# leggedrobotics/wild_visual_navigation

Measured on AMD Instinct MI355X. Metric: frames/sec (448x448 DINO-ViT-S/8 + seg + MLP train-step), higher is better.
Workload: dtype fp16 + e5m2-MX-correction linears (a w = a_h w_h + 2^-12 (a_h8 w_l8 + a_l8 w_h8); ~16 significand bits per product) + f16 attention products (two-plane q in the first six blocks), fp32 accumulate / residual (<= 1e-3 parity mode)

## Files before the change

### __graft_entry__.py

```python
import os
import sys

ROOT = os.path.dirname(os.path.abspath(__file__))
if ROOT not in sys.path:
    sys.path.insert(0, ROOT)


def build() -> None:
    from wild_visual_navigation_amd.csrc.build import build as build_lib

    path = build_lib(force=False, verbose=True)
    from oracle import build_oracle

    try:
        print("oracle:", build_oracle.build())
    except Exception as e:
        print(f"oracle: C restatement NOT built ({e}); the numpy oracle is used", file=sys.stderr)
    import wild_visual_navigation_amd
    from wild_visual_navigation_amd import _lib

    h = _lib.lib()
    print(f"libwvn_hip version {h.wvn_version()} at {path}; {len(_lib.EXPORTED_SYMBOLS)} entry points bound")


def smoke() -> None:
    import numpy as np
    import torch

    from oracle import interfaces as OI, kmeans_linear as OKL, mlp as OM, segments as OS, vit as OV
    from wild_visual_navigation_amd import ops
    from wild_visual_navigation_amd.backbone import VitBackbone
    from wild_visual_navigation_amd.feature_extractor import FeatureExtractor
    from wild_visual_navigation_amd.model import SimpleMLP
    from wild_visual_navigation_amd.traversability_estimator import MlpTrainer

    assert torch.cuda.is_available(), "smoke() needs a GPU"
    dev = torch.device("cuda:0")
    S, P, heads = 64, 8, 6
    G = S // P
    sd = OV.make_vit_state_dict("vit_small", P, pretrain_grid=4, seed=0, depth=2)
    img = torch.rand(2, 3, S, S, generator=torch.Generator().manual_seed(0))
    ref_tok = OV.vit_tokens(sd, OI.normalize(img), P, heads)[:, 1:]
    frame = torch.randint(0, 256, (1, 3, 90, 120), generator=torch.Generator().manual_seed(4), dtype=torch.uint8)
    ref_frame = OV.vit_tokens(sd, OI.dino_transform(frame.float() / 255, S), P, heads)[:, 1:]
    for prec, tol in (("exact", 1e-3), ("mixed", 1e-3), ("fp32", 1e-3), ("fp16", 8e-3), ("bf16", 6e-2)):
        bb = VitBackbone(sd, S, P, heads, device=dev, precision=prec)
        tok = bb.forward_tokens(img.to(dev)).cpu()
        err = (tok - ref_tok).abs().max().item()
        print(f"smoke: ViT tokens [{prec}] max|err| = {err:.3e} (tol {tol})")
        assert err < tol, f"backbone parity failed in {prec}: {err}"
        err = (bb.forward_tokens(frame.to(dev)).cpu() - ref_frame).abs().max().item()
        assert err < tol, f"fused ingest failed in {prec}: {err}"
    seg = OS.segment_grid(S, S, 16)[0, 0]
    dense = OI.upsample_bilinear_ac(ref_tok.reshape(2, G, G, -1).permute(0, 3, 1, 2), S)
    want = torch.stack([OS.sparsify_features(dense[b:b + 1], seg) for b in range(2)])
    got = ops.segpool_bilinear_mean(seg[None].expand(2, S, S).to(dev), ref_tok.to(dev), G, int(seg.max()) + 1).cpu()
    err = (got - want).abs().max().item()
    print(f"smoke: fused segment pooling max|err| = {err:.3e}")
    assert err < 1e-4
    code = torch.randn(1, G * G, 90, generator=torch.Generator().manual_seed(3))
    lab, _ = ops.kmeans_cosine(code.to(dev), K=5, iters=10, relabel=False)
    want_lab = OI.kmeans_cosine_labels(code[0].numpy(), 5)
    assert np.array_equal(lab[0].cpu().numpy(), want_lab), "k-means labels differ from the oracle"
    labp, _ = ops.kmeans_cosine_pixels(code.to(dev), G, 40, K=5, iters=10, relabel=False, form="direct")
    assert np.array_equal(labp[0].cpu().numpy(), OI.kmeans_cosine_labels_pixels(code[0].numpy(), G, 40, 5)), "pixel k-means labels differ"
    labl, _ = ops.kmeans_cosine_pixels(code.to(dev), G, 40, K=5, iters=10, relabel=False)
    assert np.array_equal(labl[0].cpu().numpy(), OKL.kmeans_cosine_labels_pixels_linear(code[0].numpy(), G, 40, 5)), "linear-form pixel k-means labels differ"
    print("smoke: k-means labels bit-exact (patch and pixel resolution)")
    D = 90
    g = torch.Generator().manual_seed(1)
    x = torch.randn(64, D, generator=g)
    yv = torch.rand(64, generator=g) < 0.3
    y = yv.float() * (0.5 + 0.5 * torch.rand(64, generator=g))
    model = SimpleMLP(D, [256, 32, 1], True)
    sd0 = {k: v.detach().clone() for k, v in model.state_dict().items()}
    model.to(dev)
    tr = MlpTrainer(model)
    st = OM.TrainState(sd0)
    for _ in range(3):
        got_l = tr.train_step(x.to(dev), y.to(dev), yv.to(dev)).cpu()
        want_l = OM.train_step(st, x, y, yv)
    assert abs(got_l[0].item() - want_l["loss_total"]) < 1e-5, (got_l, want_l)
    werr = max((model.state_dict()[k].cpu() - st.sd[k]).abs().max().item() for k in st.sd)
    print(f"smoke: MLP 3 Adam steps loss {got_l[0].item():.6f} (oracle {want_l['loss_total']:.6f}), max|dW| = {werr:.2e}")
    assert werr < 1e-5
    fe = FeatureExtractor(dev, segmentation_type="grid", feature_type="dino", input_size=S, backbone_type="vit_small",
                          patch_size=P, pretrained_weights=sd, precision="bf16")
    edges, feat, segm, center, _ = fe.extract(img[:1].to(dev), cell_size=16)
    assert feat.shape == (16, 384) and segm.shape == (S, S) and edges.shape[0] == 2
    print("smoke: ok")


if __name__ == "__main__":
    build()
    if len(sys.argv) > 1 and sys.argv[1] == "smoke":
        smoke()
```

### wild_visual_navigation_amd/csrc/gemm_n384_x3.hip

```cpp
#include <type_traits>

#include "common.h"
#include "wvn_internal.h"

namespace {

constexpr int NN = 384;
constexpr int NTILE = NN / 32;
constexpr int BKS = 16;
constexpr int BM = 128;
constexpr int NS = 4;
constexpr int W_PLANE = NN * BKS * 2;
constexpr int A_PLANE = BM * BKS * 2;
constexpr int A_OFF = 2 * W_PLANE;
constexpr int STAGE_BYTES = 2 * W_PLANE + 2 * A_PLANE;
constexpr int RING_BYTES = NS * STAGE_BYTES;
constexpr int STG_PITCH = 132;
constexpr int STG_BYTES = 32 * STG_PITCH * 4;
constexpr int BIAS_OFF = RING_BYTES;
constexpr int LS_OFF = BIAS_OFF + NN * 4;
constexpr int LDS_BYTES = LS_OFF + NN * 4;
constexpr int WP = 6, AP = 2;

struct N384X3Params {
// ... 259 lines not shown
    };
    __syncthreads();
#pragma unroll
    for (int j = 0; j < PD; ++j) load_a(j, j);
#pragma unroll
    for (int i0 = 0; i0 < FNS - 1; ++i0)
      if (i0 < nk) {
#pragma unroll
        for (int u = 0; u < FW; ++u) piece_w(i0, u);
      }

    f32x16_t acc[NTILE];
#pragma unroll
    for (int t = 0; t < NTILE; ++t)
#pragma unroll
      for (int r = 0; r < 16; ++r) acc[t][r] = 0.f;

    for (int ib = 0; ib < nk; ib += PD) {
#pragma unroll
      for (int jj = 0; jj < PD; ++jj) {
        const int i = ib + jj;
        long long c0 = 0, c1 = 0;
        if constexpr (TIMING) c0 = (long long)__builtin_amdgcn_s_memtime();
        asm volatile("s_waitcnt vmcnt(%0)" ::"n"((FNS - 2) * FW) : "memory");
        __builtin_amdgcn_s_barrier();
        if constexpr (TIMING) c1 = (long long)__builtin_amdgcn_s_memtime();
        __builtin_amdgcn_sched_barrier(0);
        const unsigned char* st = smem + (i % FNS) * FSTAGE;
        const bf16x8_t ah = __builtin_bit_cast(bf16x8_t, afh[jj]), al = __builtin_bit_cast(bf16x8_t, afl[jj]);
        bf16x8_t wh[2][2], wl[2][2];
#pragma unroll
        for (int t = 0; t < 2; ++t) {
          wh[0][t] = *(const bf16x8_t*)(st + rdw + t * 1024);
          wl[0][t] = *(const bf16x8_t*)(st + rdw + W_PLANE + t * 1024);
        }
#pragma unroll
        for (int pr = 0; pr < NTILE / 2; ++pr) {
          const int cur = pr & 1, nx = cur ^ 1;
          piece_w(i + FNS - 1, pr);
          if (pr + 1 < NTILE / 2) {
#pragma unroll
            for (int t = 0; t < 2; ++t) {
              wh[nx][t] = *(const bf16x8_t*)(st + rdw + (2 * pr + 2 + t) * 1024);
              wl[nx][t] = *(const bf16x8_t*)(st + rdw + W_PLANE + (2 * pr + 2 + t) * 1024);
            }
          }
#pragma unroll
          for (int term = 0; term < 3; ++term)
#pragma unroll
            for (int t = 0; t < 2; ++t) {
              const bf16x8_t w = term == 1 ? wl[cur][t] : wh[cur][t];
              const bf16x8_t a = term == 0 ? al : ah;
              acc[2 * pr + t] = __builtin_amdgcn_mfma_f32_32x32x16_bf16(w, a, acc[2 * pr + t], 0, 0, 0);
            }
#pragma unroll
          for (int n = 0; n < 6; ++n) {
            __builtin_amdgcn_sched_group_barrier(0x008, 1, 0);
            __builtin_amdgcn_sched_group_barrier(0x100, 1, 0);
            __builtin_amdgcn_sched_group_barrier(0x010, 1, 0);
            __builtin_amdgcn_sched_group_barrier(0x002, 2, 0);
          }
          __builtin_amdgcn_sched_barrier(0);
        }
        if (i + PD < nk) load_a(i + PD, jj);
        __builtin_amdgcn_sched_barrier(0);
        if constexpr (TIMING) { t_wait += c1 - c0; t_steps += (long long)__builtin_amdgcn_s_memtime() - c1; }
      }
    }
    long long e0 = 0;
    if constexpr (TIMING) e0 = (long long)__builtin_amdgcn_s_memtime();
    asm volatile("s_waitcnt vmcnt(0)" ::: "memory");
    n384_epilogue(acc, smem, wave, lane, m0w, rs_c, p.ldc, bias_l, ls_l, p.stats, p.eps, p.M, p.pos, p.npatch, p.ntok_s);
    if constexpr (TIMING) t_epi += (long long)__builtin_amdgcn_s_memtime() - e0;
  }
  if constexpr (TIMING) {
    if (lane == 0 && p.dbg) {
      long long* d = p.dbg + ((size_t)blockIdx.x * 4 + wave) * 4;
      d[0] = t_wait; d[1] = t_steps; d[2] = t_epi; d[3] = (long long)__builtin_amdgcn_s_memtime() - t_start;
    }
  }
}

constexpr int PFW = 3;
constexpr int PNS = 6;
constexpr int PRING_BYTES = PNS * FSTAGE;
constexpr int PSTG_PITCH = 68;
constexpr int PSTG_BYTES = 32 * PSTG_PITCH * 4;
constexpr int PBIAS_OFF = PRING_BYTES;
constexpr int PLS_OFF = PBIAS_OFF + NN * 4;
constexpr int PSTAT_OFF = PLS_OFF + NN * 4;
constexpr int PAIR_LDS_BYTES = PSTAT_OFF + 2 * BM * 8;
static_assert(8 * PSTG_BYTES <= PRING_BYTES && PAIR_LDS_BYTES <= 160 * 1024, "staging images must fit in the ring, the whole in the LDS");

__device__ inline void n384_pair_epilogue(const f32x16_t (&acc)[NTILE / 2], unsigned char* smem, int wave, int lane, int rg, int ch, int m0w,
                                          __amdgpu_buffer_rsrc_t rs_c, int ldc, const float* bias_l, const float* ls_l, float* stats, float eps, int M) {
  const int l31 = lane & 31, hi = lane >> 5, l15 = lane & 15, rq = lane >> 4;
  __syncthreads();
  float* stg = (float*)(smem + wave * PSTG_BYTES);
  const unsigned cvoff = (unsigned)((rq * ldc + l15 * 4) * 4);
  const int col0 = 192 * ch;
  float s1[8], s2[8];
#pragma unroll
  for (int it = 0; it < 8; ++it) { s1[it] = 0.f; s2[it] = 0.f; }
#pragma unroll
  for (int c = 0; c < 3; ++c) {
#pragma unroll
    for (int tt = 0; tt < 2; ++tt)
#pragma unroll
      for (int g = 0; g < 4; ++g) {
        const f32x16_t& a = acc[2 * c + tt];
        const f32x4_t o = {a[4 * g], a[4 * g + 1], a[4 * g + 2], a[4 * g + 3]};
        *(f32x4_t*)(stg + l31 * PSTG_PITCH + 32 * tt + 8 * g + 4 * hi) = o;
      }
    const f32x4_t b4 = *(const f32x4_t*)(bias_l + col0 + 64 * c + l15 * 4);
    const f32x4_t l4 = *(const f32x4_t*)(ls_l + col0 + 64 * c + l15 * 4);
    u32x4_t r[8];
    unsigned so_dst[8];
#pragma unroll
    for (int it = 0; it < 8; ++it) {
      so_dst[it] = __builtin_amdgcn_readfirstlane(((m0w + 4 * it) * ldc + col0 + 64 * c) * 4);
      r[it] = __builtin_amdgcn_raw_buffer_load_b128(rs_c, cvoff, so_dst[it], 0);
    }
#pragma unroll
    for (int it = 0; it < 8; ++it) {
      const f32x4_t v = *(const f32x4_t*)(stg + (4 * it + rq) * PSTG_PITCH + l15 * 4);
      u32x4_t o;
#pragma unroll
      for (int e = 0; e < 4; ++e) {
        const float y = (v[e] + b4[e]) * l4[e] + __uint_as_float(r[it][e]);
        o[e] = __float_as_uint(y);
        s1[it] += y;
        s2[it] = fmaf(y, y, s2[it]);
      }
      wvn_store_b128_guarded(o, rs_c, cvoff, so_dst[it]);
    }
  }
  if (stats) {
    float* sx = (float*)(smem + PSTAT_OFF);
    auto dpp_add = [](float v, auto ctrl) {
      constexpr int C = decltype(ctrl)::value;
      return v + __builtin_bit_cast(float, __builtin_amdgcn_update_dpp(0, __builtin_bit_cast(int, v), C, 0xf, 0xf, false));
    };
#pragma unroll
    for (int it = 0; it < 8; ++it) {
      float a = s1[it], b = s2[it];
      a = dpp_add(a, std::integral_constant<int, 0xB1>{}); b = dpp_add(b, std::integral_constant<int, 0xB1>{});
      a = dpp_add(a, std::integral_constant<int, 0x4E>{}); b = dpp_add(b, std::integral_constant<int, 0x4E>{});
      a = dpp_add(a, std::integral_constant<int, 0x141>{}); b = dpp_add(b, std::integral_constant<int, 0x141>{});
      a = dpp_add(a, std::integral_constant<int, 0x140>{}); b = dpp_add(b, std::integral_constant<int, 0x140>{});
      if (l15 == 0) *(wvn_f32x2_t*)(sx + ((size_t)ch * BM + rg * 32 + 4 * it + rq) * 2) = wvn_f32x2_t{a, b};
    }
    __syncthreads();
    if (ch == 0 && lane < 32) {
      const int m = m0w + lane;
      if (m < M) {
        const wvn_f32x2_t p0 = *(const wvn_f32x2_t*)(sx + ((size_t)rg * 32 + lane) * 2), p1 = *(const wvn_f32x2_t*)(sx + ((size_t)BM + rg * 32 + lane) * 2);
        const float a = p0[0] + p1[0], b = p0[1] + p1[1];
        const float mean = a * (1.0f / NN);
        const float var = fmaxf(b * (1.0f / NN) - mean * mean, 0.f);
        *(wvn_f32x2_t*)(stats + 2 * (size_t)m) = wvn_f32x2_t{mean, 1.0f / sqrtf(var + eps)};
      }
    }
  }
}

template <bool TIMING>
__global__ __launch_bounds__(512, 1) void gemm_n384_x3_frag_pair_kernel(N384X3Params p) {
  wvn_fp16_saturate();
  extern __shared__ __attribute__((aligned(16))) unsigned char smem[];
  const int tid = threadIdx.x, lane = tid & 63;
  const int wave = __builtin_amdgcn_readfirstlane(tid >> 6);
  const int rg = wave & 3, ch = wave >> 2;
  const int l31 = lane & 31, hi = lane >> 5;
  const int nk = p.K / BKS;
  const float* bias_l = (const float*)(smem + PBIAS_OFF);
  const float* ls_l = (const float*)(smem + PLS_OFF);
  for (int i = tid; i < NN; i += 512) {
    ((float*)(smem + PBIAS_OFF))[i] = p.bias ? p.bias[i] : 0.f;
    ((float*)(smem + PLS_OFF))[i] = p.ls ? p.ls[i] : 1.f;
  }
  const __amdgpu_buffer_rsrc_t rs_w = __builtin_amdgcn_make_buffer_rsrc((void*)p.W, 0, (unsigned)((size_t)2 * NN * p.K * 2), 0x00020000);
  const size_t mpad = (size_t)(p.M + 31) / 32 * 32;
  const __amdgpu_buffer_rsrc_t rs_a = __builtin_amdgcn_make_buffer_rsrc((void*)p.A, 0, (unsigned)((p.a_plane + mpad * p.K) * 2), 0x00020000);
  const __amdgpu_buffer_rsrc_t rs_c = __builtin_amdgcn_make_buffer_rsrc((void*)p.C, 0, (unsigned)((size_t)p.M * p.ldc * 4), 0x00020000);
  const unsigned wv0 = (unsigned)(wave * PFW * 1024 + lane * 16);
  const unsigned rdw = l31 * 32 + ((hi ^ ((l31 >> 3) & 1)) << 4) + ch * 6 * 1024;
  const unsigned a_lo_off = (unsigned)(p.a_plane * 2);

  long long t_wait = 0, t_steps = 0, t_epi = 0;
  const long long t_start = TIMING ? (long long)__builtin_amdgcn_s_memtime() : 0;
  const int nrb = (p.M + BM - 1) / BM;
  for (int rb = blockIdx.x; rb < nrb; rb += gridDim.x) {
    const int m0w = rb * BM + rg * 32;
    const unsigned a_base = __builtin_amdgcn_readfirstlane((unsigned)((size_t)(m0w >> 5) * nk * 1024));
    auto piece_w = [&](int i, int u) {
      unsigned char* st = smem + (i % PNS) * FSTAGE;
      __builtin_amdgcn_raw_ptr_buffer_load_lds(rs_w, (__attribute__((address_space(3))) void*)(st + (wave * PFW + u) * 1024), 16, wv0 + u * 1024,
                                               __builtin_amdgcn_readfirstlane((unsigned)i * FSTAGE), 0, 0);
    };
    u32x4_t afh[PD], afl[PD];
    auto load_a = [&](int i, int slot) {
      const unsigned so = __builtin_amdgcn_readfirstlane(a_base + (unsigned)i * 1024);
      afh[slot] = __builtin_amdgcn_raw_buffer_load_b128(rs_a, lane * 16, so, 0);
      afl[slot] = __builtin_amdgcn_raw_buffer_load_b128(rs_a, lane * 16, so + a_lo_off, 0);
    };
    __syncthreads();
#pragma unroll
    for (int j = 0; j < PD; ++j) load_a(j, j);
#pragma unroll
    for (int i0 = 0; i0 < PNS - 1; ++i0)
      if (i0 < nk) {
#pragma unroll
        for (int u = 0; u < PFW; ++u) piece_w(i0, u);
      }

    f32x16_t acc[NTILE / 2];
#pragma unroll
    for (int t = 0; t < NTILE / 2; ++t)
#pragma unroll
      for (int r = 0; r < 16; ++r) acc[t][r] = 0.f;

    bf16x8_t wh[2][2], wl[2][2];
    asm volatile("s_waitcnt vmcnt(%0)" ::"n"((PNS - 2) * PFW) : "memory");
    __builtin_amdgcn_s_barrier();
#pragma unroll
    for (int t = 0; t < 2; ++t) {
      wh[0][t] = *(const bf16x8_t*)(smem + rdw + t * 1024);
      wl[0][t] = *(const bf16x8_t*)(smem + rdw + W_PLANE + t * 1024);
    }
    for (int ib = 0; ib < nk; ib += PD) {
#pragma unroll
      for (int jj = 0; jj < PD; ++jj) {
        const int i = ib + jj;
        long long c0 = 0, c1 = 0;
        if constexpr (TIMING) c0 = (long long)__builtin_amdgcn_s_memtime();
        asm volatile("s_waitcnt vmcnt(%0)" ::"n"((PNS - 3) * PFW) : "memory");
        __builtin_amdgcn_s_barrier();
        if constexpr (TIMING) c1 = (long long)__builtin_amdgcn_s_memtime();
        __builtin_amdgcn_sched_barrier(0);
        const unsigned char* st = smem + (i % PNS) * FSTAGE;
        const unsigned char* st1 = smem + ((i + 1) % PNS) * FSTAGE;
        const bf16x8_t ah = __builtin_bit_cast(bf16x8_t, afh[jj]), al = __builtin_bit_cast(bf16x8_t, afl[jj]);
        const int s0 = jj & 1;
#pragma unroll
        for (int pr = 0; pr < NTILE / 4; ++pr) {
          const int cur = (s0 + pr) & 1, nx = cur ^ 1;
          piece_w(i + PNS - 1, pr);
          if (pr + 1 < NTILE / 4) {
#pragma unroll
            for (int t = 0; t < 2; ++t) {
              wh[nx][t] = *(const bf16x8_t*)(st + rdw + (2 * pr + 2 + t) * 1024);
              wl[nx][t] = *(const bf16x8_t*)(st + rdw + W_PLANE + (2 * pr + 2 + t) * 1024);
            }
          } else {
#pragma unroll
            for (int t = 0; t < 2; ++t) {
              wh[nx][t] = *(const bf16x8_t*)(st1 + rdw + t * 1024);
              wl[nx][t] = *(const bf16x8_t*)(st1 + rdw + W_PLANE + t * 1024);
            }
          }
#pragma unroll
          for (int term = 0; term < 3; ++term)
#pragma unroll
            for (int t = 0; t < 2; ++t) {
              const bf16x8_t w = term == 1 ? wl[cur][t] : wh[cur][t];
              const bf16x8_t a = term == 0 ? al : ah;
              acc[2 * pr + t] = __builtin_amdgcn_mfma_f32_32x32x16_bf16(w, a, acc[2 * pr + t], 0, 0, 0);
            }
#pragma unroll
          for (int n = 0; n < 6; ++n) {
            __builtin_amdgcn_sched_group_barrier(0x008, 1, 0);
            __builtin_amdgcn_sched_group_barrier(0x100, 1, 0);
            __builtin_amdgcn_sched_group_barrier(0x010, 1, 0);
            __builtin_amdgcn_sched_group_barrier(0x002, 2, 0);
          }
          __builtin_amdgcn_sched_barrier(0);
        }
        if (i + PD < nk) load_a(i + PD, jj);
        __builtin_amdgcn_sched_barrier(0);
        if constexpr (TIMING) { t_wait += c1 - c0; t_steps += (long long)__builtin_amdgcn_s_memtime() - c1; }
      }
    }
    long long e0 = 0;
    if constexpr (TIMING) e0 = (long long)__builtin_amdgcn_s_memtime();
    asm volatile("s_waitcnt vmcnt(0)" ::: "memory");
    n384_pair_epilogue(acc, smem, wave, lane, rg, ch, m0w, rs_c, p.ldc, bias_l, ls_l, p.stats, p.eps, p.M);
    if constexpr (TIMING) t_epi += (long long)__builtin_amdgcn_s_memtime() - e0;
  }
  if constexpr (TIMING) {
    if (lane == 0 && p.dbg && ch == 0) {
      long long* d = p.dbg + ((size_t)blockIdx.x * 4 + rg) * 4;
      d[0] = t_wait; d[1] = t_steps; d[2] = t_epi; d[3] = (long long)__builtin_amdgcn_s_memtime() - t_start;
    }
  }
}

typedef __attribute__((ext_vector_type(8))) int i32x8_t;
typedef __attribute__((ext_vector_type(8))) _Float16 f16x8_t;
constexpr int MXD = 2;
constexpr int MX_SC_ONE = 0x7f7f7f7f, MX_SC_RES = 0x73737373;

struct N384MXExtra { unsigned a_l8_off; };

template <bool TIMING, int VAR = 0>
__global__ __launch_bounds__(512, 1) void gemm_n384_mx_pair_kernel(N384X3Params p, N384MXExtra ex) {
  wvn_fp16_saturate();
  extern __shared__ __attribute__((aligned(16))) unsigned char smem[];
  const int tid = threadIdx.x, lane = tid & 63;
  const int wave = __builtin_amdgcn_readfirstlane(tid >> 6);
  const int rg = wave & 3, ch = wave >> 2;
  const int l31 = lane & 31, hi = lane >> 5;
  const int nk = p.K / BKS;
  const int nmac = p.K / 64;
  const float* bias_l = (const float*)(smem + PBIAS_OFF);
  const float* ls_l = (const float*)(smem + PLS_OFF);
  for (int i = tid; i < NN; i += 512) {
    ((float*)(smem + PBIAS_OFF))[i] = p.bias ? p.bias[i] : 0.f;
    ((float*)(smem + PLS_OFF))[i] = p.ls ? p.ls[i] : 1.f;
  }
  const __amdgpu_buffer_rsrc_t rs_w = __builtin_amdgcn_make_buffer_rsrc((void*)p.W, 0, (unsigned)((size_t)4 * NN * p.K), 0x00020000);
  const size_t mpad = (size_t)(p.M + 31) / 32 * 32;
  const __amdgpu_buffer_rsrc_t rs_a = __builtin_amdgcn_make_buffer_rsrc((void*)p.A, 0, (unsigned)(ex.a_l8_off + mpad * p.K), 0x00020000);
  const __amdgpu_buffer_rsrc_t rs_c = __builtin_amdgcn_make_buffer_rsrc((void*)p.C, 0, (unsigned)((size_t)p.M * p.ldc * 4), 0x00020000);
  const unsigned wv0 = (unsigned)(wave * PFW * 1024 + lane * 16);
  const unsigned rdw = l31 * 32 + ((hi ^ ((l31 >> 3) & 1)) << 4) + ch * 6 * 1024;

  long long t_wait = 0, t_steps = 0, t_epi = 0;
  const long long t_start = TIMING ? (long long)__builtin_amdgcn_s_memtime() : 0;
  const int nrb = (p.M + BM - 1) / BM;
  for (int rb = blockIdx.x; rb < nrb; rb += gridDim.x) {
    const int m0w = rb * BM + rg * 32;
    const unsigned a_base = __builtin_amdgcn_readfirstlane((unsigned)((size_t)(m0w >> 5) * p.K * 64));
    const unsigned a8_base = __builtin_amdgcn_readfirstlane((unsigned)((size_t)(m0w >> 5) * p.K * 32));
    auto piece_w = [&](int i, int u) {
      unsigned char* st = smem + (i % PNS) * FSTAGE;
      __builtin_amdgcn_raw_ptr_buffer_load_lds(rs_w, (__attribute__((address_space(3))) void*)(st + (wave * PFW + u) * 1024), 16, wv0 + u * 1024,
                                               __builtin_amdgcn_readfirstlane((unsigned)i * FSTAGE), 0, 0);
    };
    u32x4_t ah[MXD][4], a8[MXD][2][2];
    auto load_ah = [&](int c, int slot) {
#pragma unroll
      for (int s = 0; s < 4; ++s)
        ah[slot][s] = __builtin_amdgcn_raw_buffer_load_b128(rs_a, lane * 16, __builtin_amdgcn_readfirstlane(a_base + (unsigned)(c * 4 + s) * 1024), 0);
    };
    auto load_a8 = [&](int c, int slot) {
#pragma unroll
      for (int x = 0; x < 2; ++x)
        a8[slot][1][x] = __builtin_amdgcn_raw_buffer_load_b128(rs_a, lane * 16, __builtin_amdgcn_readfirstlane(a8_base + ex.a_l8_off + (unsigned)(c * 2 + x) * 1024), 0);
    };
    auto derive_h8 = [&](int slot) {
      typedef __attribute__((ext_vector_type(2))) short s16x2_t;
      typedef __attribute__((ext_vector_type(2))) _Float16 h2_t;
#pragma unroll
      for (int sfr = 0; sfr < 4; ++sfr) {
        uint32_t d[2] = {0, 0};
#pragma unroll
        for (int e = 0; e < 4; ++e) {
          const uint32_t pr = ah[slot][sfr][e];
          const s16x2_t o = __builtin_bit_cast(s16x2_t, d[e >> 1]);
          d[e >> 1] = __builtin_bit_cast(uint32_t, (e & 1) ? __builtin_amdgcn_cvt_scalef32_pk_bf8_f16(o, __builtin_bit_cast(h2_t, pr), 1.0f, true)
                                                           : __builtin_amdgcn_cvt_scalef32_pk_bf8_f16(o, __builtin_bit_cast(h2_t, pr), 1.0f, false));
        }
        a8[slot][0][sfr >> 1][2 * (sfr & 1)] = d[0];
        a8[slot][0][sfr >> 1][2 * (sfr & 1) + 1] = d[1];
      }
    };
    __syncthreads();
#pragma unroll
    for (int c = 0; c < MXD; ++c) {
      load_ah(c, c);
      __builtin_amdgcn_sched_barrier(0);
      load_a8(c, c);
      __builtin_amdgcn_sched_barrier(0);
    }
#pragma unroll
    for (int i0 = 0; i0 < PNS - 1; ++i0)
      if (i0 < nk) {
#pragma unroll
        for (int u = 0; u < PFW; ++u) piece_w(i0, u);
      }

    f32x16_t acc[NTILE / 2];
#pragma unroll
    for (int t = 0; t < NTILE / 2; ++t)
#pragma unroll
      for (int r = 0; r < 16; ++r) acc[t][r] = 0.f;

    u32x4_t wq[2][2][2];
    asm volatile("s_waitcnt vmcnt(%0)" ::"n"((PNS - 2) * PFW) : "memory");
    __builtin_amdgcn_s_barrier();
#pragma unroll
    for (int x = 0; x < 2; ++x)
#pragma unroll
      for (int t = 0; t < 2; ++t) wq[0][x][t] = *(const u32x4_t*)(smem + rdw + x * W_PLANE + t * 1024);
    for (int ib = 0; ib < nk; ib += 4 * MXD) {
#pragma unroll
      for (int jj = 0; jj < 4 * MXD; ++jj) {
        const int i = ib + jj;
        const int kind = jj & 3, slot = jj >> 2;
        long long c0 = 0, c1 = 0;
        if constexpr (TIMING) c0 = (long long)__builtin_amdgcn_s_memtime();
        if constexpr (VAR != 4) {
          constexpr int W3 = (PNS - 3) * PFW;
          if (jj == 0) { if (i == 0) asm volatile("s_waitcnt vmcnt(%0)" ::"n"(W3) : "memory"); else asm volatile("s_waitcnt vmcnt(%0)" ::"n"(W3 + 6) : "memory"); }
          else if (jj == 1) { if (i == 1) asm volatile("s_waitcnt vmcnt(%0)" ::"n"(W3) : "memory"); else asm volatile("s_waitcnt vmcnt(%0)" ::"n"(W3 + 2) : "memory"); }
          else if (jj == 2) { if (i == 2) asm volatile("s_waitcnt vmcnt(%0)" ::"n"(W3 + 4) : "memory"); else asm volatile("s_waitcnt vmcnt(%0)" ::"n"(W3 + 6) : "memory"); }
          else if ((jj & 3) == 0) asm volatile("s_waitcnt vmcnt(%0)" ::"n"(W3 + 6) : "memory");
          else if ((jj & 3) == 1) asm volatile("s_waitcnt vmcnt(%0)" ::"n"(W3 + 2) : "memory");
          else if ((jj & 3) == 2) asm volatile("s_waitcnt vmcnt(%0)" ::"n"(W3 + 6) : "memory");
          else asm volatile("s_waitcnt vmcnt(%0)" ::"n"(W3 + 4) : "memory");
          __builtin_amdgcn_s_barrier();
        }
        if constexpr (TIMING) c1 = (long long)__builtin_amdgcn_s_memtime();
        __builtin_amdgcn_sched_barrier(0);
        const unsigned char* st = smem + (i % PNS) * FSTAGE;
        const unsigned char* st1 = smem + ((i + 1) % PNS) * FSTAGE;
        const int s0 = jj & 1;
#pragma unroll
        for (int pr = 0; pr < NTILE / 4; ++pr) {
          const int cur = (s0 + pr) & 1, nx = cur ^ 1;
          if constexpr (!(VAR & 1) || VAR == 4) piece_w(i + PNS - 1, pr);
          const unsigned char* src = pr + 1 < NTILE / 4 ? st + (2 * pr + 2) * 1024 : st1;
#pragma unroll
          for (int x = 0; x < 2; ++x)
#pragma unroll
            for (int t = 0; t < 2; ++t) wq[nx][x][t] = *(const u32x4_t*)(src + rdw + x * W_PLANE + t * 1024);
          if (kind == 1 && pr == 0) derive_h8(slot);
          if (kind < 2) {
#pragma unroll
            for (int x = 0; x < 2; ++x)
#pragma unroll
              for (int t = 0; t < 2; ++t)
                acc[2 * pr + t] = __builtin_amdgcn_mfma_f32_32x32x16_f16(__builtin_bit_cast(f16x8_t, wq[cur][x][t]), __builtin_bit_cast(f16x8_t, ah[slot][2 * kind + x]),
                                                                         acc[2 * pr + t], 0, 0, 0);
#pragma unroll
            for (int n = 0; n < 4; ++n) {
              __builtin_amdgcn_sched_group_barrier(0x008, 1, 0);
              __builtin_amdgcn_sched_group_barrier(0x100, 1, 0);
              __builtin_amdgcn_sched_group_barrier(0x010, 1, 0);
              __builtin_amdgcn_sched_group_barrier(0x002, 2, 0);
            }
          } else {
            const u32x4_t a0 = a8[slot][kind - 2][0], a1 = a8[slot][kind - 2][1];
            const i32x8_t av = {(int)a0[0], (int)a0[1], (int)a0[2], (int)a0[3], (int)a1[0], (int)a1[1], (int)a1[2], (int)a1[3]};
#pragma unroll
            for (int t = 0; t < 2; ++t) {
              const u32x4_t w0 = wq[cur][0][t], w1 = wq[cur][1][t];
              const i32x8_t wv = {(int)w0[0], (int)w0[1], (int)w0[2], (int)w0[3], (int)w1[0], (int)w1[1], (int)w1[2], (int)w1[3]};
              acc[2 * pr + t] = __builtin_amdgcn_mfma_scale_f32_32x32x64_f8f6f4(wv, av, acc[2 * pr + t], 1, 1, 0, kind == 2 ? MX_SC_RES : MX_SC_ONE, 0,
                                                                                kind == 2 ? MX_SC_ONE : MX_SC_RES);
            }
#pragma unroll
            for (int n = 0; n < 2; ++n) {
              __builtin_amdgcn_sched_group_barrier(0x008, 1, 0);
              __builtin_amdgcn_sched_group_barrier(0x100, 2, 0);
              __builtin_amdgcn_sched_group_barrier(0x010, 1, 0);
              __builtin_amdgcn_sched_group_barrier(0x002, 4, 0);
            }
          }
          __builtin_amdgcn_sched_barrier(0);
        }
        const int c2 = (i >> 2) + MXD;
        if constexpr (!(VAR & 2) || VAR == 4) {
          if (kind == 1) load_ah(c2, slot);
          if (kind == 3) load_a8(c2, slot);
        }
        __builtin_amdgcn_sched_barrier(0);
        if constexpr (TIMING) { t_wait += c1 - c0; t_steps += (long long)__builtin_amdgcn_s_memtime() - c1; }
      }
    }
    long long e0 = 0;
    if constexpr (TIMING) e0 = (long long)__builtin_amdgcn_s_memtime();
    asm volatile("s_waitcnt vmcnt(0)" ::: "memory");
    n384_pair_epilogue(acc, smem, wave, lane, rg, ch, m0w, rs_c, p.ldc, bias_l, ls_l, p.stats, p.eps, p.M);
    if constexpr (TIMING) t_epi += (long long)__builtin_amdgcn_s_memtime() - e0;
  }
  if constexpr (TIMING) {
    if (lane == 0 && p.dbg && ch == 0) {
      long long* d = p.dbg + ((size_t)blockIdx.x * 4 + rg) * 4;
      d[0] = t_wait; d[1] = t_steps; d[2] = t_epi; d[3] = (long long)__builtin_amdgcn_s_memtime() - t_start;
    }
  }
}

int g_n384_mx_var = 0;
int g_n384_pair = 1;

int n384x3_num_cus() {
  static int n = 0;
  if (n == 0) {
    int dev = 0;
    hipDeviceProp_t prop;
    if (hipGetDevice(&dev) == hipSuccess && hipGetDeviceProperties(&prop, dev) == hipSuccess) n = prop.multiProcessorCount;
    if (n <= 0) n = 256;
  }
  return n;
}

}

int wvn_gemm_n384_x3_launch(const GemmBf16Params& g, int epi, hipStream_t st) {
  const bool patch = epi == EPI_PATCH;
  if (epi != EPI_RESID_F32 && epi != EPI_ACCUM_F32 && !patch) return WVN_ERR_ARG;
  if (patch && (!g.pos || g.npatch <= 0 || (g.npatch & 1) || g.ntok_s < g.npatch + 1 || g.ldc != NN || g.ls || (g.M % g.npatch) != 0)) return WVN_ERR_ARG;
  if (g.N != NN || g.K <= 0 || (g.K % BKS) != 0 || g.M <= 0 || !g.A || !g.A_lo || !g.W || !g.W_lo || !g.C) return WVN_ERR_ARG;
  if ((g.lda % 8) || (g.ldw % 8) || (g.ldc % 4) || g.ldw != g.K) return WVN_ERR_ARG;
  if (((uintptr_t)g.A | (uintptr_t)g.A_lo | (uintptr_t)g.W | (uintptr_t)g.W_lo | (uintptr_t)g.C) & 15) return WVN_ERR_ARG;
  if (g.A_lo <= g.A || g.W_lo <= g.W) return WVN_ERR_ARG;
  const size_t a_plane = (size_t)(g.A_lo - g.A), w_plane = (size_t)(g.W_lo - g.W);
  const size_t c_rows = patch ? (size_t)(g.M / g.npatch) * g.ntok_s : (size_t)g.M;
  if ((a_plane + (size_t)g.M * g.lda) * 2 >= (1ull << 32) || c_rows * g.ldc * 4 >= (1ull << 32) || (w_plane + (size_t)NN * g.ldw) * 2 >= (1ull << 32))
    return WVN_ERR_ARG;
  N384X3Params p{};
  p.A = g.A; p.a_plane = a_plane; p.lda = g.lda; p.W = g.W; p.w_plane = w_plane; p.ldw = g.ldw; p.bias = g.bias; p.ls = g.ls;
  p.C = (float*)g.C; p.ldc = g.ldc; p.M = g.M; p.K = g.K; p.dbg = g.dbg; p.stats = g.ln_stats_out; p.eps = g.ln_eps;
  if (patch) { p.pos = g.pos; p.npatch = g.npatch; p.ntok_s = g.ntok_s; p.c_rows = (int)c_rows; p.stats = nullptr; }
  static LdsOptIn lds_opt_in;
  if (const int rc = lds_opt_in(LDS_BYTES, (const void*)gemm_n384_x3_kernel<false>, (const void*)gemm_n384_x3_kernel<true>)) return rc;
  const int ncu = n384x3_num_cus(), nrb = ceil_div(g.M, BM);
  const int grid = nrb < ncu ? nrb : ncu;
  if (p.dbg) hipLaunchKernelGGL(gemm_n384_x3_kernel<true>, dim3(grid), dim3(256), LDS_BYTES, st, p);
  else hipLaunchKernelGGL(gemm_n384_x3_kernel<false>, dim3(grid), dim3(256), LDS_BYTES, st, p);
  WVN_LAUNCH_CHECK();
  return WVN_OK;
}

int wvn_gemm_n384_x3_frag_launch(const GemmBf16Params& g, int epi, hipStream_t st) {
  if (epi != EPI_RESID_F32 && epi != EPI_ACCUM_F32) return WVN_ERR_ARG;
  if (g.N != NN || g.K <= 0 || (g.K % (BKS * PD)) != 0 || g.M <= 0 || !g.A || !g.A_lo || !g.W || !g.C || (g.ldc % 4)) return WVN_ERR_ARG;
  if (((uintptr_t)g.A | (uintptr_t)g.A_lo | (uintptr_t)g.W | (uintptr_t)g.C) & 15) return WVN_ERR_ARG;
  if (g.A_lo <= g.A) return WVN_ERR_ARG;
  const size_t a_plane = (size_t)(g.A_lo - g.A), mpad = (size_t)(g.M + 31) / 32 * 32;
  if ((a_plane + mpad * g.K) * 2 >= (1ull << 32) || (size_t)g.M * g.ldc * 4 >= (1ull << 32) || (size_t)2 * NN * g.K * 2 >= (1ull << 31)) return WVN_ERR_ARG;
  N384X3Params p{};
  p.A = g.A; p.a_plane = a_plane; p.lda = g.K; p.W = g.W; p.w_plane = 0; p.ldw = g.K; p.bias = g.bias; p.ls = g.ls;
  p.C = (float*)g.C; p.ldc = g.ldc; p.M = g.M; p.K = g.K; p.dbg = g.dbg; p.stats = g.ln_stats_out; p.eps = g.ln_eps;
  static LdsOptIn lds_opt_in;
  if (const int rc = lds_opt_in(PAIR_LDS_BYTES, (const void*)gemm_n384_x3_frag_kernel<false>, (const void*)gemm_n384_x3_frag_kernel<true>,
                                (const void*)gemm_n384_x3_frag_pair_kernel<false>, (const void*)gemm_n384_x3_frag_pair_kernel<true>)) return rc;
  const int ncu = n384x3_num_cus(), nrb = ceil_div(g.M, BM);
  const int grid = nrb < ncu ? nrb : ncu;
  if (g_n384_pair) {
    if (p.dbg) hipLaunchKernelGGL(gemm_n384_x3_frag_pair_kernel<true>, dim3(grid), dim3(512), PAIR_LDS_BYTES, st, p);
    else hipLaunchKernelGGL(gemm_n384_x3_frag_pair_kernel<false>, dim3(grid), dim3(512), PAIR_LDS_BYTES, st, p);
  } else if (p.dbg) hipLaunchKernelGGL(gemm_n384_x3_frag_kernel<true>, dim3(grid), dim3(256), LDS_BYTES, st, p);
  else hipLaunchKernelGGL(gemm_n384_x3_frag_kernel<false>, dim3(grid), dim3(256), LDS_BYTES, st, p);
  WVN_LAUNCH_CHECK();
  return WVN_OK;
}
int wvn_gemm_n384_mx_launch(const GemmBf16Params& g, int epi, hipStream_t st) {
  if (epi != EPI_RESID_F32 && epi != EPI_ACCUM_F32) return WVN_ERR_ARG;
  if (g.N != NN || g.K <= 0 || (g.K % 128) != 0 || g.M <= 0 || !g.A || !g.A_lo || !g.W || !g.C || (g.ldc % 4)) return WVN_ERR_ARG;
  if (((uintptr_t)g.A | (uintptr_t)g.A_lo | (uintptr_t)g.W | (uintptr_t)g.C) & 15) return WVN_ERR_ARG;
  const size_t mpad = (size_t)(g.M + 31) / 32 * 32;
  const uintptr_t a0 = (uintptr_t)g.A, al = (uintptr_t)g.A_lo;
  if (al < a0 + mpad * g.K * 2) return WVN_ERR_ARG;
  const uintptr_t top = al + mpad * g.K;
  if (top - a0 >= (1ull << 32) || (size_t)g.M * g.ldc * 4 >= (1ull << 32) || (size_t)4 * NN * g.K >= (1ull << 31)) return WVN_ERR_ARG;
  N384X3Params p{};
  p.A = g.A; p.a_plane = 0; p.lda = g.K; p.W = g.W; p.w_plane = 0; p.ldw = g.K; p.bias = g.bias; p.ls = g.ls;
  p.C = (float*)g.C; p.ldc = g.ldc; p.M = g.M; p.K = g.K; p.dbg = g.dbg; p.stats = g.ln_stats_out; p.eps = g.ln_eps;
  N384MXExtra ex{(unsigned)(al - a0)};
  static LdsOptIn lds_opt_in;
  if (const int rc = lds_opt_in(PAIR_LDS_BYTES, (const void*)gemm_n384_mx_pair_kernel<false>, (const void*)gemm_n384_mx_pair_kernel<true>,
                                (const void*)gemm_n384_mx_pair_kernel<true, 1>, (const void*)gemm_n384_mx_pair_kernel<true, 2>,
                                (const void*)gemm_n384_mx_pair_kernel<true, 3>, (const void*)gemm_n384_mx_pair_kernel<true, 4>)) return rc;
  const int ncu = n384x3_num_cus(), nrb = ceil_div(g.M, BM);
  const int grid = nrb < ncu ? nrb : ncu;
  if (p.dbg && g_n384_mx_var == 1) hipLaunchKernelGGL((gemm_n384_mx_pair_kernel<true, 1>), dim3(grid), dim3(512), PAIR_LDS_BYTES, st, p, ex);
  else if (p.dbg && g_n384_mx_var == 2) hipLaunchKernelGGL((gemm_n384_mx_pair_kernel<true, 2>), dim3(grid), dim3(512), PAIR_LDS_BYTES, st, p, ex);
  else if (p.dbg && g_n384_mx_var == 3) hipLaunchKernelGGL((gemm_n384_mx_pair_kernel<true, 3>), dim3(grid), dim3(512), PAIR_LDS_BYTES, st, p, ex);
  else if (p.dbg && g_n384_mx_var == 4) hipLaunchKernelGGL((gemm_n384_mx_pair_kernel<true, 4>), dim3(grid), dim3(512), PAIR_LDS_BYTES, st, p, ex);
  else if (p.dbg) hipLaunchKernelGGL(gemm_n384_mx_pair_kernel<true>, dim3(grid), dim3(512), PAIR_LDS_BYTES, st, p, ex);
  else hipLaunchKernelGGL(gemm_n384_mx_pair_kernel<false>, dim3(grid), dim3(512), PAIR_LDS_BYTES, st, p, ex);
  WVN_LAUNCH_CHECK();
  return WVN_OK;
}
void wvn_gemm_n384_x3_set_pair(int on) {
  if (on >= 16) { g_n384_mx_var = on - 16; return; }
  g_n384_pair = on ? 1 : 0;
}
```

Before: 882.5.

## Overlap next row-block A/W prefetch and residual loads with MX pair GEMM epilogue

Restructures the MX pair GEMM's persistent row-block loop so the last k-trip is peeled. That trip prefetches the residual tile into registers, preloads the first W stages for the next row block into ring slots, and issues the next block's A loads from inside a new custom epilogue after each column group. The epilogue stages through unused ring slots, adds bias/layer-scale/residual and computes LayerNorm stats. This is meant to hide the epilogue's global residual reads and the next tile's pipeline fill latency. It adds many registers and complex vmcnt accounting, and only fully applies when nk is a multiple of the stage count.

```diff
diff --git a/__graft_entry__.py b/__graft_entry__.py
--- a/__graft_entry__.py
+++ b/__graft_entry__.py
@@ -72,6 +72,7 @@
     x = torch.randn(64, D, generator=g)
     yv = torch.rand(64, generator=g) < 0.3
     y = yv.float() * (0.5 + 0.5 * torch.rand(64, generator=g))
+    torch.manual_seed(0)
     model = SimpleMLP(D, [256, 32, 1], True)
     sd0 = {k: v.detach().clone() for k, v in model.state_dict().items()}
     model.to(dev)
diff --git a/wild_visual_navigation_amd/csrc/gemm_n384_x3.hip b/wild_visual_navigation_amd/csrc/gemm_n384_x3.hip
--- a/wild_visual_navigation_amd/csrc/gemm_n384_x3.hip
+++ b/wild_visual_navigation_amd/csrc/gemm_n384_x3.hip
@@ -585,6 +585,78 @@
 
 struct N384MXExtra { unsigned a_l8_off; };
 
+constexpr int MX_STG_OFF = 3 * FSTAGE;
+static_assert(MX_STG_OFF + 8 * PSTG_BYTES <= PRING_BYTES, "the MX staging images must fit in ring slots 3 - 5");
+template <class AfterGroup>
+__device__ inline void n384_mx_pair_epilogue(const f32x16_t (&acc)[NTILE / 2], const u32x4_t (&res)[24], unsigned char* smem, int wave, int lane, int rg, int ch,
+                                             int m0w, __amdgpu_buffer_rsrc_t rs_c, int ldc, const float* bias_l, const float* ls_l, float* stats, float eps, int M,
+                                             AfterGroup&& after_group) {
+  const int l31 = lane & 31, hi = lane >> 5, l15 = lane & 15, rq = lane >> 4;
+  float* stg = (float*)(smem + MX_STG_OFF + wave * PSTG_BYTES);
+  const unsigned cvoff = (unsigned)((rq * ldc + l15 * 4) * 4);
+  const int col0 = 192 * ch;
+  float s1[8], s2[8];
+#pragma unroll
+  for (int it = 0; it < 8; ++it) { s1[it] = 0.f; s2[it] = 0.f; }
+#pragma unroll
+  for (int c = 0; c < 3; ++c) {
+#pragma unroll
+    for (int tt = 0; tt < 2; ++tt)
+#pragma unroll
+      for (int g = 0; g < 4; ++g) {
+        const f32x16_t& a = acc[2 * c + tt];
+        const f32x4_t o = {a[4 * g], a[4 * g + 1], a[4 * g + 2], a[4 * g + 3]};
+        *(f32x4_t*)(stg + l31 * PSTG_PITCH + 32 * tt + 8 * g + 4 * hi) = o;
+      }
+    const f32x4_t b4 = *(const f32x4_t*)(bias_l + col0 + 64 * c + l15 * 4);
+    const f32x4_t l4 = *(const f32x4_t*)(ls_l + col0 + 64 * c + l15 * 4);
+#pragma unroll
+    for (int it = 0; it < 8; ++it) {
+      const unsigned so = __builtin_amdgcn_readfirstlane(((m0w + 4 * it) * ldc + col0 + 64 * c) * 4);
+      const f32x4_t v = *(const f32x4_t*)(stg + (4 * it + rq) * PSTG_PITCH + l15 * 4);
+      u32x4_t o;
+#pragma unroll
+      for (int e = 0; e < 4; ++e) {
+        const float y = (v[e] + b4[e]) * l4[e] + __uint_as_float(res[8 * c + it][e]);
+        o[e] = __float_as_uint(y);
+        s1[it] += y;
+        s2[it] = fmaf(y, y, s2[it]);
+      }
+      wvn_store_b128_guarded(o, rs_c, cvoff, so);
+    }
+    if (c == 0) after_group(std::integral_constant<int, 0>{});
+    if (c == 1) after_group(std::integral_constant<int, 1>{});
+  }
+  if (stats) {
+    float* sx = (float*)(smem + PSTAT_OFF);
+    auto dpp_add = [](float v, auto ctrl) {
+      constexpr int C = decltype(ctrl)::value;
+      return v + __builtin_bit_cast(float, __builtin_amdgcn_update_dpp(0, __builtin_bit_cast(int, v), C, 0xf, 0xf, false));
+    };
+#pragma unroll
+    for (int it = 0; it < 8; ++it) {
+      float a = s1[it], b = s2[it];
+      a = dpp_add(a, std::integral_constant<int, 0xB1>{}); b = dpp_add(b, std::integral_constant<int, 0xB1>{});
+      a = dpp_add(a, std::integral_constant<int, 0x4E>{}); b = dpp_add(b, std::integral_constant<int, 0x4E>{});
+      a = dpp_add(a, std::integral_constant<int, 0x141>{}); b = dpp_add(b, std::integral_constant<int, 0x141>{});
+      a = dpp_add(a, std::integral_constant<int, 0x140>{}); b = dpp_add(b, std::integral_constant<int, 0x140>{});
+      if (l15 == 0) *(wvn_f32x2_t*)(sx + ((size_t)ch * BM + rg * 32 + 4 * it + rq) * 2) = wvn_f32x2_t{a, b};
+    }
+    __syncthreads();
+    if (ch == 0 && lane < 32) {
+      const int m = m0w + lane;
+      if (m < M) {
+        const wvn_f32x2_t p0 = *(const wvn_f32x2_t*)(sx + ((size_t)rg * 32 + lane) * 2), p1 = *(const wvn_f32x2_t*)(sx + ((size_t)BM + rg * 32 + lane) * 2);
+        const float a = p0[0] + p1[0], b = p0[1] + p1[1];
+        const float mean = a * (1.0f / NN);
+        const float var = fmaxf(b * (1.0f / NN) - mean * mean, 0.f);
+        *(wvn_f32x2_t*)(stats + 2 * (size_t)m) = wvn_f32x2_t{mean, 1.0f / sqrtf(var + eps)};
+      }
+    }
+  }
+}
+
+
 template <bool TIMING, int VAR = 0>
 __global__ __launch_bounds__(512, 1) void gemm_n384_mx_pair_kernel(N384X3Params p, N384MXExtra ex) {
   wvn_fp16_saturate();
@@ -607,29 +679,51 @@
   const __amdgpu_buffer_rsrc_t rs_c = __builtin_amdgcn_make_buffer_rsrc((void*)p.C, 0, (unsigned)((size_t)p.M * p.ldc * 4), 0x00020000);
   const unsigned wv0 = (unsigned)(wave * PFW * 1024 + lane * 16);
   const unsigned rdw = l31 * 32 + ((hi ^ ((l31 >> 3) & 1)) << 4) + ch * 6 * 1024;
+  const unsigned cvoff = (unsigned)(((lane >> 4) * p.ldc + (lane & 15) * 4) * 4);
+  const bool pre = (nk % PNS) == 0;
 
   long long t_wait = 0, t_steps = 0, t_epi = 0;
   const long long t_start = TIMING ? (long long)__builtin_amdgcn_s_memtime() : 0;
   const int nrb = (p.M + BM - 1) / BM;
+  unsigned a_base = 0, a8_base = 0;
+  auto set_a_base = [&](int rb_) {
+    const size_t R = (size_t)(rb_ * (BM / 32) + rg);
+    a_base = __builtin_amdgcn_readfirstlane((unsigned)(R * p.K * 64));
+    a8_base = __builtin_amdgcn_readfirstlane((unsigned)(R * p.K * 32));
+  };
+  u32x4_t ah[MXD][4], a8[MXD][2][2];
+  auto load_ah = [&](int c, int slot) {
+#pragma unroll
+    for (int s = 0; s < 4; ++s)
+      ah[slot][s] = __builtin_amdgcn_raw_buffer_load_b128(rs_a, lane * 16, __builtin_amdgcn_readfirstlane(a_base + (unsigned)(c * 4 + s) * 1024), 0);
+  };
+  auto load_a8 = [&](int c, int slot) {
+#pragma unroll
+    for (int x = 0; x < 2; ++x)
+      a8[slot][1][x] = __builtin_amdgcn_raw_buffer_load_b128(rs_a, lane * 16, __builtin_amdgcn_readfirstlane(a8_base + ex.a_l8_off + (unsigned)(c * 2 + x) * 1024), 0);
+  };
+  auto load_a_head = [&](int rb_, int c) {
+    set_a_base(rb_);
+    __builtin_amdgcn_sched_barrier(0);
+    load_ah(c, c);
+    __builtin_amdgcn_sched_barrier(0);
+    load_a8(c, c);
+    __builtin_amdgcn_sched_barrier(0);
+  };
+  static_assert(MXD == 2, "one 64-k step of A behind each of the epilogue's first two column groups");
+  load_a_head(blockIdx.x, 0);
+  load_a_head(blockIdx.x, 1);
   for (int rb = blockIdx.x; rb < nrb; rb += gridDim.x) {
     const int m0w = rb * BM + rg * 32;
-    const unsigned a_base = __builtin_amdgcn_readfirstlane((unsigned)((size_t)(m0w >> 5) * p.K * 64));
-    const unsigned a8_base = __builtin_amdgcn_readfirstlane((unsigned)((size_t)(m0w >> 5) * p.K * 32));
-    auto piece_w = [&](int i, int u) {
+    auto piece_w = [&](int i, int u, int src) {
       unsigned char* st = smem + (i % PNS) * FSTAGE;
       __builtin_amdgcn_raw_ptr_buffer_load_lds(rs_w, (__attribute__((address_space(3))) void*)(st + (wave * PFW + u) * 1024), 16, wv0 + u * 1024,
-                                               __builtin_amdgcn_readfirstlane((unsigned)i * FSTAGE), 0, 0);
-    };
-    u32x4_t ah[MXD][4], a8[MXD][2][2];
-    auto load_ah = [&](int c, int slot) {
-#pragma unroll
-      for (int s = 0; s < 4; ++s)
-        ah[slot][s] = __builtin_amdgcn_raw_buffer_load_b128(rs_a, lane * 16, __builtin_amdgcn_readfirstlane(a_base + (unsigned)(c * 4 + s) * 1024), 0);
-    };
-    auto load_a8 = [&](int c, int slot) {
-#pragma unroll
-      for (int x = 0; x < 2; ++x)
-        a8[slot][1][x] = __builtin_amdgcn_raw_buffer_load_b128(rs_a, lane * 16, __builtin_amdgcn_readfirstlane(a8_base + ex.a_l8_off + (unsigned)(c * 2 + x) * 1024), 0);
+                                               __builtin_amdgcn_readfirstlane((unsigned)src * FSTAGE), 0, 0);
+    };
+    const bool full = !pre || rb == (int)blockIdx.x;
+    u32x4_t res[24];
+    auto load_res = [&](int q) {
+      res[q] = __builtin_amdgcn_raw_buffer_load_b128(rs_c, cvoff, __builtin_amdgcn_readfirstlane(((m0w + 4 * (q & 7)) * p.ldc + 192 * ch + 64 * (q >> 3)) * 4), 0);
     };
     auto derive_h8 = [&](int slot) {
       typedef __attribute__((ext_vector_type(2))) short s16x2_t;
@@ -650,17 +744,10 @@
     };
     __syncthreads();
 #pragma unroll
-    for (int c = 0; c < MXD; ++c) {
-      load_ah(c, c);
-      __builtin_amdgcn_sched_barrier(0);
-      load_a8(c, c);
-      __builtin_amdgcn_sched_barrier(0);
-    }
-#pragma unroll
     for (int i0 = 0; i0 < PNS - 1; ++i0)
-      if (i0 < nk) {
-#pragma unroll
-        for (int u = 0; u < PFW; ++u) piece_w(i0, u);
+      if (i0 < nk && (full || i0 >= 3)) {
+#pragma unroll
+        for (int u = 0; u < PFW; ++u) piece_w(i0, u, i0);
       }
 
     f32x16_t acc[NTILE / 2];
@@ -670,13 +757,16 @@
       for (int r = 0; r < 16; ++r) acc[t][r] = 0.f;
 
     u32x4_t wq[2][2][2];
-    asm volatile("s_waitcnt vmcnt(%0)" ::"n"((PNS - 2) * PFW) : "memory");
-    __builtin_amdgcn_s_barrier();
+    if (full) {
+      asm volatile("s_waitcnt vmcnt(%0)" ::"n"((PNS - 2) * PFW) : "memory");
+      __builtin_amdgcn_s_barrier();
+    }
 #pragma unroll
     for (int x = 0; x < 2; ++x)
 #pragma unroll
       for (int t = 0; t < 2; ++t) wq[0][x][t] = *(const u32x4_t*)(smem + rdw + x * W_PLANE + t * 1024);
-    for (int ib = 0; ib < nk; ib += 4 * MXD) {
+    auto trip = [&](const int ib, auto last_c) __attribute__((always_inline)) {
+      constexpr bool LAST = decltype(last_c)::value;
 #pragma unroll
       for (int jj = 0; jj < 4 * MXD; ++jj) {
         const int i = ib + jj;
@@ -685,13 +775,13 @@
         if constexpr (TIMING) c0 = (long long)__builtin_amdgcn_s_memtime();
         if constexpr (VAR != 4) {
           constexpr int W3 = (PNS - 3) * PFW;
-          if (jj == 0) { if (i == 0) asm volatile("s_waitcnt vmcnt(%0)" ::"n"(W3) : "memory"); else asm volatile("s_waitcnt vmcnt(%0)" ::"n"(W3 + 6) : "memory"); }
-          else if (jj == 1) { if (i == 1) asm volatile("s_waitcnt vmcnt(%0)" ::"n"(W3) : "memory"); else asm volatile("s_waitcnt vmcnt(%0)" ::"n"(W3 + 2) : "memory"); }
+          if (jj == 0) { if (i == 0) { if (full) asm volatile("s_waitcnt vmcnt(%0)" ::"n"(W3) : "memory"); } else asm volatile("s_waitcnt vmcnt(%0)" ::"n"(W3 + 6) : "memory"); }
+          else if (jj == 1) { if (i == 1) { if (full) asm volatile("s_waitcnt vmcnt(%0)" ::"n"(W3) : "memory"); } else asm volatile("s_waitcnt vmcnt(%0)" ::"n"(W3 + 2) : "memory"); }
           else if (jj == 2) { if (i == 2) asm volatile("s_waitcnt vmcnt(%0)" ::"n"(W3 + 4) : "memory"); else asm volatile("s_waitcnt vmcnt(%0)" ::"n"(W3 + 6) : "memory"); }
-          else if ((jj & 3) == 0) asm volatile("s_waitcnt vmcnt(%0)" ::"n"(W3 + 6) : "memory");
-          else if ((jj & 3) == 1) asm volatile("s_waitcnt vmcnt(%0)" ::"n"(W3 + 2) : "memory");
+          else if ((jj & 3) == 0) { if constexpr (LAST) asm volatile("s_waitcnt vmcnt(%0)" ::"n"(W3 + 8) : "memory"); else asm volatile("s_waitcnt vmcnt(%0)" ::"n"(W3 + 6) : "memory"); }
+          else if ((jj & 3) == 1) { if constexpr (LAST) asm volatile("s_waitcnt vmcnt(%0)" ::"n"(W3 + 4) : "memory"); else asm volatile("s_waitcnt vmcnt(%0)" ::"n"(W3 + 2) : "memory"); }
           else if ((jj & 3) == 2) asm volatile("s_waitcnt vmcnt(%0)" ::"n"(W3 + 6) : "memory");
-          else asm volatile("s_waitcnt vmcnt(%0)" ::"n"(W3 + 4) : "memory");
+          else { if constexpr (LAST) asm volatile("s_waitcnt vmcnt(%0)" ::"n"(W3 + 6) : "memory"); else asm volatile("s_waitcnt vmcnt(%0)" ::"n"(W3 + 4) : "memory"); }
           __builtin_amdgcn_s_barrier();
         }
         if constexpr (TIMING) c1 = (long long)__builtin_amdgcn_s_memtime();
@@ -702,7 +792,10 @@
 #pragma unroll
         for (int pr = 0; pr < NTILE / 4; ++pr) {
           const int cur = (s0 + pr) & 1, nx = cur ^ 1;
-          if constexpr (!(VAR & 1) || VAR == 4) piece_w(i + PNS - 1, pr);
+          if constexpr (!(VAR & 1) || VAR == 4) {
+            if (LAST && jj >= 3 && jj < 6) piece_w(i + PNS - 1, pr, pre ? jj - 3 : i + PNS - 1);
+            else piece_w(i + PNS - 1, pr, i + PNS - 1);
+          }
           const unsigned char* src = pr + 1 < NTILE / 4 ? st + (2 * pr + 2) * 1024 : st1;
 #pragma unroll
           for (int x = 0; x < 2; ++x)
@@ -744,18 +837,29 @@
           __builtin_amdgcn_sched_barrier(0);
         }
         const int c2 = (i >> 2) + MXD;
-        if constexpr (!(VAR & 2) || VAR == 4) {
+        if constexpr (LAST) {
+          if (kind == 1) { load_res(8 * slot); load_res(8 * slot + 1); load_res(8 * slot + 2); load_res(8 * slot + 3); }
+          if (kind == 2) { load_res(8 * slot + 4); load_res(8 * slot + 5); }
+          if (kind == 3) { load_res(8 * slot + 6); load_res(8 * slot + 7); }
+        } else if constexpr (!(VAR & 2) || VAR == 4) {
           if (kind == 1) load_ah(c2, slot);
           if (kind == 3) load_a8(c2, slot);
         }
         __builtin_amdgcn_sched_barrier(0);
         if constexpr (TIMING) { t_wait += c1 - c0; t_steps += (long long)__builtin_amdgcn_s_memtime() - c1; }
       }
-    }
+    };
+    for (int ib = 0; ib < nk - 4 * MXD; ib += 4 * MXD) trip(ib, std::false_type{});
+    trip(nk - 4 * MXD, std::true_type{});
     long long e0 = 0;
     if constexpr (TIMING) e0 = (long long)__builtin_amdgcn_s_memtime();
-    asm volatile("s_waitcnt vmcnt(0)" ::: "memory");
-    n384_pair_epilogue(acc, smem, wave, lane, rg, ch, m0w, rs_c, p.ldc, bias_l, ls_l, p.stats, p.eps, p.M);
+#pragma unroll
+    for (int q = 16; q < 24; ++q) load_res(q);
+    __builtin_amdgcn_sched_barrier(0);
+    asm volatile("s_waitcnt vmcnt(10)" ::: "memory");
+    __syncthreads();
+    n384_mx_pair_epilogue(acc, res, smem, wave, lane, rg, ch, m0w, rs_c, p.ldc, bias_l, ls_l, p.stats, p.eps, p.M,
+                          [&](auto c) { load_a_head(rb + (int)gridDim.x, decltype(c)::value); });
     if constexpr (TIMING) t_epi += (long long)__builtin_amdgcn_s_memtime() - e0;
   }
   if constexpr (TIMING) {
```

New measurement: 888.1 (median of 6 runs). Within noise of the previous version (+0.6%).
